# KC-decoder/Multimodal-Brain-Pattern-Identification_XAI

Hardware: AMD Instinct MI355X
Metric: samples/sec train (multimodal SpectrogramCNN+EEGNet fusion, B=64/GPU, 4x128x256 spectro + 10000x19 EEG) (higher is better)
Workload: dtype bf16

## Files before the change

multimodal-brain-pattern-identification_xai_amd/csrc/conv3x3_mfma.hip:

```cpp
#include <stdlib.h>
#include "bx_common.h"
#include <string.h>

typedef __attribute__((ext_vector_type(8))) short bf16x8;
typedef __attribute__((ext_vector_type(4))) float f32x4;
typedef unsigned int u32x4 __attribute__((ext_vector_type(4)));
typedef unsigned int u32x2 __attribute__((ext_vector_type(2)));

static inline int mfma_ck(int Ci) { return Ci < 64 ? Ci : 64; }
static inline int mfma_ks(int ck) { return (9 * ck + 31) / 32; }

int bx_conv3x3_mfma_supported(int Ci, int Co, int dtype) {
  if (dtype != BX_BF16) return 0;
  if (!(Ci == 8 || Ci == 16 || Ci == 32 || (Ci >= 64 && Ci % 64 == 0))) return 0;
  return (Co >= 16 && Co % 16 == 0) || (Co == 8 && (Ci == 16 || Ci == 32));
}
static inline int mfma_ow(int O_p) { return O_p < 16 ? 16 : O_p; }
extern "C" size_t bx_conv3x3_packed_mfma_bytes(int I_p, int O_p) {
  if (!bx_conv3x3_mfma_supported(I_p, O_p, BX_BF16)) return 0;
  const int ck = mfma_ck(I_p);
  return (size_t)(I_p / ck) * mfma_ks(ck) * mfma_ow(O_p) * 32 * sizeof(bf16_t);
}

__global__ void k_pack_mfma(const float* __restrict__ w, bf16_t* __restrict__ wp, int Cout, int Cin, int I_p, int O_p, int tf,
// ... 173 lines not shown

__device__ __forceinline__ unsigned char relu_bits(u32x2 v) {
  const uint32_t h[4] = {v.x & 0xffffu, v.x >> 16, v.y & 0xffffu, v.y >> 16};
  unsigned b = 0;
#pragma unroll
  for (int r = 0; r < 4; ++r) b |= (h[r] != 0u && h[r] < 0x8000u) ? (1u << r) : 0u;
  return (unsigned char)b;
}
template <int CTRL> __device__ __forceinline__ float dpp16(float v) {
  return __int_as_float(__builtin_amdgcn_update_dpp(0, __float_as_int(v), CTRL, 0xf, 0xf, false));
}
__device__ __forceinline__ float row16_sum(float v) {
  v += dpp16<0xB1>(v); v += dpp16<0x4E>(v); v += dpp16<0x124>(v); v += dpp16<0x128>(v);
  return v;
}
template <int MP, int NC, int TPR, typename PixFn>
__device__ __forceinline__ void conv_pool_tiles(const f32x4 (&q)[MP][NC], const BxConvPoolEpi& pe, const __amdgpu_buffer_rsrc_t& pres, int Co,
                                                int co_base, PixFn pix, float (&st)[2][NC][4]) {
  const int lane = threadIdx.x & 63, g = lane >> 4, li = lane & 15;
  const __amdgpu_buffer_rsrc_t rres = __builtin_amdgcn_make_buffer_rsrc(pe.route, 0, pe.route ? pe.route_bytes : 0u, 0x00020000);
#pragma unroll
  for (int i = 0; i < MP; ++i) {
    if ((i / TPR) % 2) continue;
    int bimg, oy, ox;
    pix(i, bimg, oy, ox);
    const bool own = !(li & 1) && (oy >> 1) < pe.Ho && (ox >> 1) < pe.Wo;
    const uint32_t po = own ? (uint32_t)(((((bimg * pe.Ho + (oy >> 1)) * pe.Wo + (ox >> 1)) * Co) + co_base + 4 * g) * 2) : 0x80000000u;
#pragma unroll
    for (int n = 0; n < NC; ++n) {
      float v[4];
      uint32_t code = 0;
#pragma unroll
      for (int r = 0; r < 4; ++r) {
        const float t0 = q[i][n][r], b0 = q[i + TPR][n][r];
        const float t1 = dpp16<0xB1>(t0), b1 = dpp16<0xB1>(b0);
        v[r] = pe.pool == BX_POOL_MAX ? fmaxf(fmaxf(t0, t1), fmaxf(b0, b1)) : 0.25f * (t0 + t1 + b0 + b1);
        if (pe.route) {
          uint32_t nib;
          if (pe.pool == BX_POOL_MAX) {
            nib = t0 == v[r] ? 1u : t1 == v[r] ? 2u : b0 == v[r] ? 4u : 8u;
            nib = v[r] > 0.f ? nib : 0u;
          } else {
            nib = (t0 > 0.f ? 1u : 0u) | (t1 > 0.f ? 2u : 0u) | (b0 > 0.f ? 4u : 0u) | (b1 > 0.f ? 8u : 0u);
          }
          code |= nib << (4 * r);
        }
      }
      const uint32_t lo = pack2bf(v[0], v[1]), hi = pack2bf(v[2], v[3]);
      __builtin_amdgcn_raw_buffer_store_b64((u32x2){lo, hi}, pres, po + (uint32_t)(n * 32), 0, 0);
      __builtin_amdgcn_raw_buffer_store_b16((short)code, rres, own ? (po >> 2) + (uint32_t)(n * 8) : 0x80000000u, 0, 0);
      if (own) {
        const float w[4] = {__uint_as_float(lo << 16), __uint_as_float(lo & 0xffff0000u), __uint_as_float(hi << 16), __uint_as_float(hi & 0xffff0000u)};
#pragma unroll
        for (int r = 0; r < 4; ++r) { st[0][n][r] += w[r]; st[1][n][r] += w[r] * w[r]; }
      }
    }
  }
}
template <int NC>
__device__ __forceinline__ void conv_pool_finish(float (&st)[2][NC][4], const BxConvPoolEpi& pe, int co_base, char* lds) {
  if (!pe.want_stats) return;
  const int wave = threadIdx.x >> 6, lane = threadIdx.x & 63, g = lane >> 4, li = lane & 15;
  constexpr int CW = NC * 16;
#pragma unroll
  for (int k = 0; k < 2; ++k)
// ... 169 lines not shown
      for (int n = 0; n < NC; ++n) {
        const float v[4] = {fmaxf(acc[i][n][0] + bz[n].x, 0.f), fmaxf(acc[i][n][1] + bz[n].y, 0.f), fmaxf(acc[i][n][2] + bz[n].z, 0.f),
                            fmaxf(acc[i][n][3] + bz[n].w, 0.f)};
        const u32x2 out = {pack2bf(v[0], v[1]), pack2bf(v[2], v[3])};
        if (pe.store_y) __builtin_amdgcn_raw_buffer_store_b64(out, yres, offs[i][n], 0, 0);
        acc[i][n] = (f32x4){__uint_as_float(out.x << 16), __uint_as_float(out.x & 0xffff0000u), __uint_as_float(out.y << 16),
                            __uint_as_float(out.y & 0xffff0000u)};
      }
    const uint32_t p_bytes = (uint32_t)((size_t)gx / (tiles_x * tiles_y) * IMGS * pe.Ho * pe.Wo * Co * 2);
    const __amdgpu_buffer_rsrc_t pres = __builtin_amdgcn_make_buffer_rsrc(pe.pooled, 0, p_bytes, 0x00020000);
    float st[2][NC][4];
#pragma unroll
    for (int n = 0; n < NC; ++n)
#pragma unroll
      for (int r = 0; r < 4; ++r) st[0][n][r] = st[1][n][r] = 0.f;
    conv_pool_tiles<MP, NC, TPR>(acc, pe, pres, Co, co_base, [&](int i, int& bimg, int& oy, int& ox) {
      const int t = wave * MP + i, img = t / TPI, tl = t % TPI;
      bimg = b + img; oy = y0 + tl / TPR; ox = x0 + (tl % TPR) * 16 + li;
    }, st);
    conv_pool_finish<NC>(st, pe, co_base, lds);
    return;
  }
  if (mask_src) {
    if (mbits) {
#pragma unroll
      for (int i = 0; i < MP; ++i)
#pragma unroll
        for (int n = 0; n < NCW; ++n) mk[i][n].x = __builtin_amdgcn_raw_buffer_load_b8(mres, offs[i][n] >> 3, 0, 0);
    } else {
#pragma unroll
      for (int i = 0; i < MP; ++i)
#pragma unroll
        for (int n = 0; n < NCW; ++n) mk[i][n] = __builtin_amdgcn_raw_buffer_load_b64(mres, offs[i][n], 0, 0);
// ... 169 lines not shown
      for (int n = 0; n < NCW; ++n) {
        const float v[4] = {fmaxf(acc[i][n][0] + bz[n].x, 0.f), fmaxf(acc[i][n][1] + bz[n].y, 0.f), fmaxf(acc[i][n][2] + bz[n].z, 0.f),
                            fmaxf(acc[i][n][3] + bz[n].w, 0.f)};
        const u32x2 out = {pack2bf(v[0], v[1]), pack2bf(v[2], v[3])};
        if (pe.store_y) __builtin_amdgcn_raw_buffer_store_b64(out, yres, offs[i] + (uint32_t)(n * 32), 0, 0);
        acc[i][n] = (f32x4){__uint_as_float(out.x << 16), __uint_as_float(out.x & 0xffff0000u), __uint_as_float(out.y << 16),
                            __uint_as_float(out.y & 0xffff0000u)};
      }
    const uint32_t p_bytes = (uint32_t)((size_t)gridDim.x / (tiles_x * tiles_y) * IMGS * pe.Ho * pe.Wo * Co * 2);
    const __amdgpu_buffer_rsrc_t pres = __builtin_amdgcn_make_buffer_rsrc(pe.pooled, 0, p_bytes, 0x00020000);
    float st[2][NCW][4];
#pragma unroll
    for (int n = 0; n < NCW; ++n)
#pragma unroll
      for (int r = 0; r < 4; ++r) st[0][n][r] = st[1][n][r] = 0.f;
    conv_pool_tiles<MPT, NCW, TPR>(acc, pe, pres, Co, co_base, [&](int i, int& bimg, int& oy, int& ox) {
      const int img = i / TPI, tl = i % TPI;
      bimg = b + img; oy = y0 + tl / TPR; ox = x0 + (tl % TPR) * 16 + li;
    }, st);
    if (pe.want_stats) {
#pragma unroll
      for (int k = 0; k < 2; ++k)
#pragma unroll
        for (int n = 0; n < NCW; ++n)
#pragma unroll
          for (int r = 0; r < 4; ++r) st[k][n][r] = row16_sum(st[k][n][r]);
      if (li == 0) {
#pragma unroll
        for (int k = 0; k < 2; ++k)
#pragma unroll
          for (int n = 0; n < NCW; ++n)
            *reinterpret_cast<float4*>(pe.tree.rows + ((size_t)blockIdx.x * 2 + k) * pe.tree.ld + co_base + n * 16 + 4 * g) =
                make_float4(st[k][n][0], st[k][n][1], st[k][n][2], st[k][n][3]);
// ... 30 lines not shown
        for (int r = 0; r < 4; ++r) v[r] = (mm[r] != 0u && mm[r] < 0x8000u) ? v[r] : 0.f;
      }
      if (addend) {
        const u32x2 a2 = ad[i][n];
        v[0] += __uint_as_float(a2.x << 16); v[1] += __uint_as_float(a2.x & 0xffff0000u);
        v[2] += __uint_as_float(a2.y << 16); v[3] += __uint_as_float(a2.y & 0xffff0000u);
      }
      const u32x2 out = {pack2bf(v[0], v[1]), pack2bf(v[2], v[3])};
      __builtin_amdgcn_raw_buffer_store_b64(out, yres, offs[i] + (uint32_t)(n * 32), 0, 0);
    }
  }
  BX_CSTAMP(6);
}

template <int CK, int NC, int TW, bool POOL = false, bool C8 = false>
__global__ __launch_bounds__(256, (CK == 16 && NC == 1 && TW == 32 && !POOL) ? 4 : 1) void k_conv_mfma_p(const bf16_t* __restrict__ x, const bf16_t* __restrict__ wp, const float* __restrict__ bias,
    const bf16_t* __restrict__ mask_src, const bf16_t* __restrict__ addend, bf16_t* __restrict__ y,
    int H, int W, int Co, int relu, int tiles_x, int tiles_y, int ntiles, uint32_t x_bytes, BxConvPoolEpi pe, WgradRedList red, int nred) {
  constexpr int TH = 8, HWID = TW + 2, HH = TH + 2, CKB = CK * 2, NCH = CK / 8, KS = (9 * CK + 31) / 32;
  constexpr int MP = TH * TW / 64, TPR = TW / 16;
  constexpr int NU = HH * HWID * NCH, NR = (NU + 255) / 256;
  extern __shared__ __attribute__((aligned(16))) char lds[];
  if ((int)blockIdx.x < nred) {
    if (blockIdx.y == 0) wgrad_reduce_list(red, (int)blockIdx.x, reinterpret_cast<float4*>(lds));
    return;
  }
  const int first_tile = (int)blockIdx.x - nred, tile_stride = (int)gridDim.x - nred;
  const int co_base = blockIdx.y * (NC * 16);
  const int wave = threadIdx.x >> 6, lane = threadIdx.x & 63, g = lane >> 4, li = lane & 15;
  uint4 rv[NR];
  const __amdgpu_buffer_rsrc_t xres = __builtin_amdgcn_make_buffer_rsrc((void*)x, 0, x_bytes, 0x00020000);
// ... 22 lines not shown
  const uint32_t y_bytes = (uint32_t)((size_t)(ntiles / (tiles_x * tiles_y)) * H * W * Co * 2);
  const __amdgpu_buffer_rsrc_t yres = __builtin_amdgcn_make_buffer_rsrc((void*)y, 0, y_bytes, 0x00020000);
  const bool mbits = (relu & 2) != 0;
  const __amdgpu_buffer_rsrc_t mres = __builtin_amdgcn_make_buffer_rsrc((void*)(mask_src ? mask_src : y), 0, mbits ? y_bytes / 8 : y_bytes, 0x00020000);
  const __amdgpu_buffer_rsrc_t ares = __builtin_amdgcn_make_buffer_rsrc((void*)(addend ? addend : y), 0, y_bytes, 0x00020000);
  const uint32_t lane_rel = (uint32_t)((li * Co + co_base + 4 * g) * 2);
  const int Cw = C8 ? 16 : Co;
  const bool ch_ok = C8 ? g < 2 : true;
  float4 bz[NC];
#pragma unroll
  for (int n = 0; n < NC; ++n)
    bz[n] = bias && ch_ok ? *reinterpret_cast<const float4*>(bias + co_base + n * 16 + 4 * g) : make_float4(0.f, 0.f, 0.f, 0.f);
  if (first_tile < ntiles) fetch(first_tile);
  float st[2][NC][4];
  __amdgpu_buffer_rsrc_t pres = yres;
  if constexpr (POOL) {
    conv_pool_transpose_w1x1(pe, Co);
    pres = __builtin_amdgcn_make_buffer_rsrc(pe.pooled, 0, (uint32_t)((size_t)(ntiles / (tiles_x * tiles_y)) * pe.Ho * pe.Wo * Co * 2), 0x00020000);
#pragma unroll
    for (int n = 0; n < NC; ++n)
#pragma unroll
      for (int r = 0; r < 4; ++r) st[0][n][r] = st[1][n][r] = 0.f;
  }
  for (int tile = first_tile; tile < ntiles; tile += tile_stride) {
    const int tx = tile % tiles_x, ty = (tile / tiles_x) % tiles_y, b = tile / (tiles_x * tiles_y);
    const int y0 = ty * TH, x0 = tx * TW;
    __syncthreads();
#pragma unroll
    for (int k = 0; k < NR; ++k) {
      const int u = threadIdx.x + k * 256;
      if (u < NU) {
// ... 25 lines not shown
      const int c = (q0 % CK) / 8;
      const bool valid = tap < 9;
      if (!valid) tap = 0;
      const int dy = tap / 3, dx = tap - 3 * dy;
#pragma unroll
      for (int i = 0; i < MP; ++i) {
        const int t = wave * MP + i;
        const int p = (t / TPR + dy) * HWID + (t % TPR) * 16 + li + dx;
        bf16x8 bv = *reinterpret_cast<const bf16x8*>(lds + p * CKB + 16 * lds_chunk<CK>(c, p));
        if (!valid) bv = (bf16x8){0, 0, 0, 0, 0, 0, 0, 0};
#pragma unroll
        for (int n = 0; n < NC; ++n) acc[i][n] = __builtin_amdgcn_mfma_f32_16x16x32_bf16(a[s % 3][n], bv, acc[i][n], 0, 0, 0);
      }
    }
    const uint32_t tile_o = (uint32_t)((((b * H + y0) * W + x0) * Co) * 2) + lane_rel;
    uint32_t offs[MP][NC];
    u32x2 mk[MP][NC], ad[MP][NC];
#pragma unroll
    for (int i = 0; i < MP; ++i) {
      const int t = wave * MP + i;
      const int oy = y0 + t / TPR, ox = x0 + (t % TPR) * 16 + li;
      const bool inb = oy < H && ox < W && ch_ok;
      const uint32_t orow = tile_o + (uint32_t)((((t / TPR) * W + (t % TPR) * 16) * Co) * 2);
#pragma unroll
      for (int n = 0; n < NC; ++n) offs[i][n] = inb ? orow + (uint32_t)(n * 32) : 0x80000000u;
    }
    if constexpr (POOL) {
#pragma unroll
      for (int i = 0; i < MP; ++i)
#pragma unroll
        for (int n = 0; n < NC; ++n) {
          const float v[4] = {fmaxf(acc[i][n][0] + bz[n].x, 0.f), fmaxf(acc[i][n][1] + bz[n].y, 0.f), fmaxf(acc[i][n][2] + bz[n].z, 0.f),
                              fmaxf(acc[i][n][3] + bz[n].w, 0.f)};
          const u32x2 out = {pack2bf(v[0], v[1]), pack2bf(v[2], v[3])};
          if (pe.store_y) __builtin_amdgcn_raw_buffer_store_b64(out, yres, offs[i][n], 0, 0);
          acc[i][n] = (f32x4){__uint_as_float(out.x << 16), __uint_as_float(out.x & 0xffff0000u), __uint_as_float(out.y << 16),
                              __uint_as_float(out.y & 0xffff0000u)};
        }
      conv_pool_tiles<MP, NC, TPR>(acc, pe, pres, Co, co_base, [&](int i, int& bimg, int& oy, int& ox) {
        const int t = wave * MP + i;
        bimg = b; oy = y0 + t / TPR; ox = x0 + (t % TPR) * 16 + li;
      }, st);
      continue;
    }
    if (mask_src) {
      if (mbits) {
#pragma unroll
        for (int i = 0; i < MP; ++i)
#pragma unroll
          for (int n = 0; n < NC; ++n) mk[i][n].x = __builtin_amdgcn_raw_buffer_load_b8(mres, offs[i][n] >> 3, 0, 0);
      } else {
#pragma unroll
        for (int i = 0; i < MP; ++i)
#pragma unroll
          for (int n = 0; n < NC; ++n) mk[i][n] = __builtin_amdgcn_raw_buffer_load_b64(mres, offs[i][n], 0, 0);
      }
    }
    if (addend) {
// ... 22 lines not shown
          for (int r = 0; r < 4; ++r) v[r] = (mm[r] != 0u && mm[r] < 0x8000u) ? v[r] : 0.f;
        }
        if (addend) {
          const u32x2 a2 = ad[i][n];
          v[0] += __uint_as_float(a2.x << 16); v[1] += __uint_as_float(a2.x & 0xffff0000u);
          v[2] += __uint_as_float(a2.y << 16); v[3] += __uint_as_float(a2.y & 0xffff0000u);
        }
        const u32x2 out = {pack2bf(v[0], v[1]), pack2bf(v[2], v[3])};
        __builtin_amdgcn_raw_buffer_store_b64(out, yres, offs[i][n], 0, 0);
      }
    }
  }
  if constexpr (POOL) conv_pool_finish<NC>(st, pe, co_base, lds);
}

template <bool STORE1>
__global__ __launch_bounds__(256, 4) void k_conv12_mfma(const bf16_t* __restrict__ x, const bf16_t* __restrict__ wp1, const float* __restrict__ bias1,
    const bf16_t* __restrict__ wp2, const float* __restrict__ bias2, bf16_t* __restrict__ y1, bf16_t* __restrict__ y2,
    unsigned char* __restrict__ m1, unsigned char* __restrict__ m2, int H, int W, int tiles_x, int tiles_y, int ntiles, uint32_t x_bytes) {
  constexpr int TH = 8, TW = 32, XW = TW + 4, XH = TH + 4, YW = TW + 2, YH = TH + 2, NX = XH * XW, NY = YH * YW;
  constexpr int NR = (NX + 255) / 256, NT1 = (NY + 15) / 16, MP = TH * TW / 64, TPR = TW / 16, KS1 = 3, KS2 = 5;
  extern __shared__ __attribute__((aligned(16))) char lds[];
  char* xs = lds;
  char* y1s = lds + NX * 16;
  const int wave = threadIdx.x >> 6, lane = threadIdx.x & 63, g = lane >> 4, li = lane & 15;
  const __amdgpu_buffer_rsrc_t xres = __builtin_amdgcn_make_buffer_rsrc((void*)x, 0, x_bytes, 0x00020000);
  int hpy[NR], hpx[NR];
  uint32_t hrel[NR];
#pragma unroll
  for (int k = 0; k < NR; ++k) {
    const int u = threadIdx.x + k * 256;
    hpy[k] = u < NX ? u / XW - 2 : -100000;
    hpx[k] = u % XW - 2;
    hrel[k] = (uint32_t)(((u / XW - 2) * W + (u % XW - 2)) * 8) * 2u;
  }
  uint4 rv[NR];
  auto fetch = [&](int tile) {
    const int tx = tile % tiles_x, ty = (tile / tiles_x) % tiles_y, b = tile / (tiles_x * tiles_y);
    const int y0 = ty * TH, x0 = tx * TW;
    const uint32_t tbase = (uint32_t)(((b * H + y0) * W + x0) * 8) * 2u;
#pragma unroll
    for (int k = 0; k < NR; ++k) {
      const bool ok = (unsigned)(y0 + hpy[k]) < (unsigned)H && (unsigned)(x0 + hpx[k]) < (unsigned)W;
      const u32x4 v = __builtin_amdgcn_raw_buffer_load_b128(xres, ok ? tbase + hrel[k] : 0x80000000u, 0, 0);
      rv[k] = make_uint4(v.x, v.y, v.z, v.w);
    }
  };
  const uint32_t y_bytes = (uint32_t)((size_t)(ntiles / (tiles_x * tiles_y)) * H * W * 16 * 2);
  const __amdgpu_buffer_rsrc_t y1res = __builtin_amdgcn_make_buffer_rsrc((void*)(STORE1 ? y1 : y2), 0, y_bytes, 0x00020000);
  const __amdgpu_buffer_rsrc_t y2res = __builtin_amdgcn_make_buffer_rsrc((void*)y2, 0, y_bytes, 0x00020000);
  const __amdgpu_buffer_rsrc_t m1res = __builtin_amdgcn_make_buffer_rsrc((void*)(STORE1 && m1 ? (void*)m1 : (void*)y2), 0, STORE1 && m1 ? y_bytes / 8 : 0u, 0x00020000);
  const __amdgpu_buffer_rsrc_t m2res = __builtin_amdgcn_make_buffer_rsrc((void*)(STORE1 && m2 ? (void*)m2 : (void*)y2), 0, STORE1 && m2 ? y_bytes / 8 : 0u, 0x00020000);
  bf16x8 a1[KS1], a2[KS2];
#pragma unroll
  for (int s = 0; s < KS1; ++s) a1[s] = *reinterpret_cast<const bf16x8*>(wp1 + ((size_t)s * 16 + li) * 32 + 8 * g);
#pragma unroll
  for (int s = 0; s < KS2; ++s) a2[s] = *reinterpret_cast<const bf16x8*>(wp2 + ((size_t)s * 16 + li) * 32 + 8 * g);
  const float4 b1z = *reinterpret_cast<const float4*>(bias1 + 4 * g), b2z = *reinterpret_cast<const float4*>(bias2 + 4 * g);
  const int first_tile = (int)blockIdx.x, tile_stride = (int)gridDim.x;
  if (first_tile < ntiles) fetch(first_tile);
  for (int tile = first_tile; tile < ntiles; tile += tile_stride) {
    const int tx = tile % tiles_x, ty = (tile / tiles_x) % tiles_y, b = tile / (tiles_x * tiles_y);
    const int y0 = ty * TH, x0 = tx * TW;
    __syncthreads();
#pragma unroll
    for (int k = 0; k < NR; ++k) {
      const int u = threadIdx.x + k * 256;
      if (u < NX) *reinterpret_cast<uint4*>(xs + u * 16) = rv[k];
    }
    __syncthreads();
    if (tile + tile_stride < ntiles) fetch(tile + tile_stride);
#pragma unroll 2
    for (int it = 0; it < (NT1 + 3) / 4; ++it) {
      const int t = wave + 4 * it;
      if (t >= NT1) break;
      const int p = 16 * t + li, pc = p < NY ? p : NY - 1;
      const int r = pc / YW, c = pc - r * YW;
      f32x4 acc = {0.f, 0.f, 0.f, 0.f};
#pragma unroll
      for (int s = 0; s < KS1; ++s) {
        int tap = 4 * s + g;
        const bool valid = tap < 9;
        if (!valid) tap = 0;
        const int dy = tap / 3, dx = tap - 3 * dy;
        bf16x8 bv = *reinterpret_cast<const bf16x8*>(xs + ((r + dy) * XW + c + dx) * 16);
        if (!valid) bv = (bf16x8){0, 0, 0, 0, 0, 0, 0, 0};
        acc = __builtin_amdgcn_mfma_f32_16x16x32_bf16(a1[s], bv, acc, 0, 0, 0);
      }
      const int iy = y0 - 1 + r, ix = x0 - 1 + c;
      const bool inside = p < NY && (unsigned)iy < (unsigned)H && (unsigned)ix < (unsigned)W;
      const float v0 = inside ? fmaxf(acc[0] + b1z.x, 0.f) : 0.f, v1 = inside ? fmaxf(acc[1] + b1z.y, 0.f) : 0.f;
      const float v2 = inside ? fmaxf(acc[2] + b1z.z, 0.f) : 0.f, v3 = inside ? fmaxf(acc[3] + b1z.w, 0.f) : 0.f;
      const u32x2 out = {pack2bf(v0, v1), pack2bf(v2, v3)};
      if (p < NY) *reinterpret_cast<u32x2*>(y1s + p * 32 + 8 * g) = out;
      if constexpr (STORE1) {
        const bool own = inside && r >= 1 && r <= TH && c >= 1 && c <= TW;
        const uint32_t off = own ? (uint32_t)((((b * H + iy) * W + ix) * 16 + 4 * g) * 2) : 0x80000000u;
        __builtin_amdgcn_raw_buffer_store_b64(out, y1res, off, 0, 0);
        __builtin_amdgcn_raw_buffer_store_b8(relu_bits(out), m1res, off >> 3, 0, 0);
      }
    }
    __syncthreads();
    f32x4 acc2[MP];
#pragma unroll
    for (int i = 0; i < MP; ++i) acc2[i] = (f32x4){0.f, 0.f, 0.f, 0.f};
#pragma unroll
    for (int s = 0; s < KS2; ++s) {
      const int q0 = s * 32 + 8 * g;
      int tap = q0 / 16;
      const int c8 = (q0 % 16) / 8;
      const bool valid = tap < 9;
      if (!valid) tap = 0;
      const int dy = tap / 3, dx = tap - 3 * dy;
#pragma unroll
      for (int i = 0; i < MP; ++i) {
        const int t = wave * MP + i;
        const int p = (t / TPR + dy) * YW + (t % TPR) * 16 + li + dx;
        bf16x8 bv = *reinterpret_cast<const bf16x8*>(y1s + p * 32 + 16 * c8);
        if (!valid) bv = (bf16x8){0, 0, 0, 0, 0, 0, 0, 0};
        acc2[i] = __builtin_amdgcn_mfma_f32_16x16x32_bf16(a2[s], bv, acc2[i], 0, 0, 0);
      }
    }
#pragma unroll
    for (int i = 0; i < MP; ++i) {
      const int t = wave * MP + i;
      const int oy = y0 + t / TPR, ox = x0 + (t % TPR) * 16 + li;
      const bool inb = oy < H && ox < W;
      const uint32_t off = inb ? (uint32_t)((((b * H + oy) * W + ox) * 16 + 4 * g) * 2) : 0x80000000u;
      const u32x2 out = {pack2bf(fmaxf(acc2[i][0] + b2z.x, 0.f), fmaxf(acc2[i][1] + b2z.y, 0.f)),
                         pack2bf(fmaxf(acc2[i][2] + b2z.z, 0.f), fmaxf(acc2[i][3] + b2z.w, 0.f))};
      __builtin_amdgcn_raw_buffer_store_b64(out, y2res, off, 0, 0);
      if constexpr (STORE1) __builtin_amdgcn_raw_buffer_store_b8(relu_bits(out), m2res, off >> 3, 0, 0);
    }
  }
}
template <int C0, int C1, bool STORE1>
__global__ __launch_bounds__(256, C1 <= 32 ? 4 : 2) void k_conv12b_mfma(const bf16_t* __restrict__ x, const bf16_t* __restrict__ wp1, const float* __restrict__ bias1,
    const bf16_t* __restrict__ wp2, const float* __restrict__ bias2, bf16_t* __restrict__ y1, bf16_t* __restrict__ y2,
    unsigned char* __restrict__ m1, unsigned char* __restrict__ m2, int H, int W, int tiles_x, int tiles_y, int ntiles, uint32_t x_bytes) {
  constexpr int TH = 8, TW = 32, XW = TW + 4, XH = TH + 4, YW = TW + 2, YH = TH + 2, NX = XH * XW, NY = YH * YW;
  constexpr int NCH0 = C0 / 8, XB = C0 * 2, YB = C1 * 2, NU = NX * NCH0, NR = (NU + 255) / 256, NT1 = (NY + 15) / 16, MP = TH * TW / 64, TPR = TW / 16;
  constexpr int KS1 = (9 * C0 + 31) / 32, KS2 = (9 * C1 + 31) / 32, NC = C1 / 16;
  extern __shared__ __attribute__((aligned(16))) char lds[];
  char* xs = lds;
  char* y1s = lds + NX * XB;
  const int wave = threadIdx.x >> 6, lane = threadIdx.x & 63, g = lane >> 4, li = lane & 15;
  const __amdgpu_buffer_rsrc_t xres = __builtin_amdgcn_make_buffer_rsrc((void*)x, 0, x_bytes, 0x00020000);
  const uint32_t y_bytes = (uint32_t)((size_t)(ntiles / (tiles_x * tiles_y)) * H * W * C1 * 2);
  const __amdgpu_buffer_rsrc_t y1res = __builtin_amdgcn_make_buffer_rsrc((void*)(STORE1 ? y1 : y2), 0, y_bytes, 0x00020000);
  const __amdgpu_buffer_rsrc_t y2res = __builtin_amdgcn_make_buffer_rsrc((void*)y2, 0, y_bytes, 0x00020000);
  const __amdgpu_buffer_rsrc_t m1res = __builtin_amdgcn_make_buffer_rsrc((void*)(STORE1 && m1 ? (void*)m1 : (void*)y2), 0, STORE1 && m1 ? y_bytes / 8 : 0u, 0x00020000);
  const __amdgpu_buffer_rsrc_t m2res = __builtin_amdgcn_make_buffer_rsrc((void*)(STORE1 && m2 ? (void*)m2 : (void*)y2), 0, STORE1 && m2 ? y_bytes / 8 : 0u, 0x00020000);
  const int tile = (int)blockIdx.x;
  const int tx = tile % tiles_x, ty = (tile / tiles_x) % tiles_y, b = tile / (tiles_x * tiles_y);
  const int y0 = ty * TH, x0 = tx * TW;
  {
    const uint32_t tbase = (uint32_t)(((b * H + y0) * W + x0) * C0) * 2u;
// ... 47 lines not shown
#pragma unroll
      for (int n = 0; n < NC; ++n) acc[n] = __builtin_amdgcn_mfma_f32_16x16x32_bf16(a1[s % 3][n], bv, acc[n], 0, 0, 0);
    }
    const int iy = y0 - 1 + r, ix = x0 - 1 + c;
    const bool inside = p < NY && (unsigned)iy < (unsigned)H && (unsigned)ix < (unsigned)W;
    const bool own = inside && r >= 1 && r <= TH && c >= 1 && c <= TW;
    const uint32_t goff = own ? (uint32_t)((((b * H + iy) * W + ix) * C1 + 4 * g) * 2) : 0x80000000u;
#pragma unroll
    for (int n = 0; n < NC; ++n) {
      const float v0 = inside ? fmaxf(acc[n][0] + b1z[n].x, 0.f) : 0.f, v1 = inside ? fmaxf(acc[n][1] + b1z[n].y, 0.f) : 0.f;
      const float v2 = inside ? fmaxf(acc[n][2] + b1z[n].z, 0.f) : 0.f, v3 = inside ? fmaxf(acc[n][3] + b1z[n].w, 0.f) : 0.f;
      const u32x2 out = {pack2bf(v0, v1), pack2bf(v2, v3)};
      if (p < NY) *reinterpret_cast<u32x2*>(y1s + p * YB + 16 * lds_chunk<C1>(2 * n + (g >> 1), p) + 8 * (g & 1)) = out;
      if constexpr (STORE1) {
        __builtin_amdgcn_raw_buffer_store_b64(out, y1res, own ? goff + (uint32_t)(n * 32) : 0x80000000u, 0, 0);
        __builtin_amdgcn_raw_buffer_store_b8(relu_bits(out), m1res, own ? (goff + (uint32_t)(n * 32)) >> 3 : 0x80000000u, 0, 0);
      }
    }
  }
  __syncthreads();
  f32x4 acc2[MP][NC];
#pragma unroll
  for (int i = 0; i < MP; ++i)
#pragma unroll
    for (int n = 0; n < NC; ++n) acc2[i][n] = (f32x4){0.f, 0.f, 0.f, 0.f};
  bf16x8 a2[3][NC];
  auto load_a2 = [&](int s_, bf16x8 (&dst)[NC]) {
#pragma unroll
    for (int n = 0; n < NC; ++n) dst[n] = *reinterpret_cast<const bf16x8*>(wp2 + ((size_t)s_ * C1 + n * 16 + li) * 32 + 8 * g);
  };
  load_a2(0, a2[0]);
// ... 17 lines not shown
#pragma unroll
      for (int n = 0; n < NC; ++n) acc2[i][n] = __builtin_amdgcn_mfma_f32_16x16x32_bf16(a2[s % 3][n], bv, acc2[i][n], 0, 0, 0);
    }
  }
#pragma unroll
  for (int i = 0; i < MP; ++i) {
    const int t = wave * MP + i;
    const int oy = y0 + t / TPR, ox = x0 + (t % TPR) * 16 + li;
    const bool inb = oy < H && ox < W;
    const uint32_t off = inb ? (uint32_t)((((b * H + oy) * W + ox) * C1 + 4 * g) * 2) : 0x80000000u;
#pragma unroll
    for (int n = 0; n < NC; ++n) {
      const u32x2 out = {pack2bf(fmaxf(acc2[i][n][0] + b2z[n].x, 0.f), fmaxf(acc2[i][n][1] + b2z[n].y, 0.f)),
                         pack2bf(fmaxf(acc2[i][n][2] + b2z[n].z, 0.f), fmaxf(acc2[i][n][3] + b2z[n].w, 0.f))};
      __builtin_amdgcn_raw_buffer_store_b64(out, y2res, inb ? off + (uint32_t)(n * 32) : 0x80000000u, 0, 0);
      if constexpr (STORE1) __builtin_amdgcn_raw_buffer_store_b8(relu_bits(out), m2res, inb ? (off + (uint32_t)(n * 32)) >> 3 : 0x80000000u, 0, 0);
    }
  }
}
extern "C" int bx_conv3x3_pair_supported(int C0_p, int C1, int C2, int dtype) {
  return dtype == BX_BF16 && ((C0_p == 8 && C1 == 16 && C2 == 16) || (C0_p == 16 && C1 == 32 && C2 == 32) ||
                              (C0_p == 32 && C1 == 64 && C2 == 64));
}
extern "C" int bx_conv3x3_pair(const void* x, const void* packed1_mfma, const float* bias1, const void* packed2_mfma, const float* bias2,
                               void* y1, void* y2, unsigned char* mask1, unsigned char* mask2, int B, int H, int W, int C0_p, int C1, int C2,
                               int dtype, bxStream stream) {
  BX_REQUIRE(y1 || (!mask1 && !mask2), "bx_conv3x3_pair: the ReLU bit masks are written together with y1 (training passes)");
  BX_REQUIRE(x && packed1_mfma && bias1 && packed2_mfma && bias2 && y2 && B > 0 && H > 0 && W > 0, "bx_conv3x3_pair: bad arguments");
  BX_REQUIRE(bx_conv3x3_pair_supported(C0_p, C1, C2, dtype), "bx_conv3x3_pair: built for bf16 storage, 8 (padded) -> 16 -> 16, 16 -> 32 -> 32 or 32 -> 64 -> 64 channels (got %d -> %d -> %d)",
             C0_p, C1, C2);
  BX_REQUIRE((size_t)B * H * W * C1 * 2 < ((size_t)1 << 31), "bx_conv3x3_pair: an activation tensor of 2 GiB or more is not supported");
  const int tiles_x = (W + 31) / 32, tiles_y = (H + 7) / 8;
  const long long ntiles = (long long)tiles_x * tiles_y * B;
  BX_REQUIRE(ntiles < (1ll << 31), "bx_conv3x3_pair: too many tiles");
  constexpr int gx_cap = 2048;
  const int gx = ntiles < gx_cap ? (int)ntiles : gx_cap;
  if (C1 >= 32) {
    const size_t lds2 = (size_t)12 * 36 * C0_p * 2 + (size_t)10 * 34 * C1 * 2;
    const uint32_t xb2 = (uint32_t)((size_t)B * H * W * C0_p * 2);
    auto go = [&](auto kern) -> int {
      static bool attr_done = false;
      if (lds2 > 64 * 1024 && !attr_done) {
        if (hipFuncSetAttribute((const void*)kern, hipFuncAttributeMaxDynamicSharedMemorySize, (int)lds2) != hipSuccess)
          BX_FAIL(BX_EHIP, "bx_conv3x3_pair: cannot reserve %zu bytes of LDS", lds2);
        attr_done = true;
      }
      hipLaunchKernelGGL(kern, dim3((unsigned)ntiles), dim3(256), lds2, (hipStream_t)stream, (const bf16_t*)x, (const bf16_t*)packed1_mfma, bias1,
                         (const bf16_t*)packed2_mfma, bias2, (bf16_t*)y1, (bf16_t*)y2, y1 ? mask1 : (unsigned char*)nullptr,
                         y1 ? mask2 : (unsigned char*)nullptr, H, W, tiles_x, tiles_y, (int)ntiles, xb2);
      BX_CHECK_LAUNCH("bx_conv3x3_pair (stages 2-3)");
      return BX_OK;
    };
    if (C1 == 32) return y1 ? go(k_conv12b_mfma<16, 32, true>) : go(k_conv12b_mfma<16, 32, false>);
    return y1 ? go(k_conv12b_mfma<32, 64, true>) : go(k_conv12b_mfma<32, 64, false>);
  }
  const size_t lds = (size_t)12 * 36 * 16 + (size_t)10 * 34 * 32;
  const uint32_t xb = (uint32_t)((size_t)B * H * W * 8 * 2);
  if (y1)
    hipLaunchKernelGGL((k_conv12_mfma<true>), dim3((unsigned)gx), dim3(256), lds, (hipStream_t)stream, (const bf16_t*)x, (const bf16_t*)packed1_mfma, bias1,
                       (const bf16_t*)packed2_mfma, bias2, (bf16_t*)y1, (bf16_t*)y2, mask1, mask2, H, W, tiles_x, tiles_y, (int)ntiles, xb);
  else
    hipLaunchKernelGGL((k_conv12_mfma<false>), dim3((unsigned)gx), dim3(256), lds, (hipStream_t)stream, (const bf16_t*)x, (const bf16_t*)packed1_mfma, bias1,
                       (const bf16_t*)packed2_mfma, bias2, (bf16_t*)nullptr, (bf16_t*)y2, (unsigned char*)nullptr, (unsigned char*)nullptr, H, W, tiles_x, tiles_y, (int)ntiles, xb);
  BX_CHECK_LAUNCH("bx_conv3x3_pair");
  return BX_OK;
}

template <int NC>
static int pool_tree_shape(BxConvPoolEpi* pe, int grid_x, int ygroups, int Co) {
  pe->tree.nrows = grid_x; pe->tree.Cw = NC * 16; pe->tree.ld = Co;
  bx_stat_tree_shape(grid_x, &pe->tree.G, &pe->tree.ngroups);
  if (!pe->want_stats) return BX_OK;
  if (grid_x > pe->tree_max_rows) pe->tree.cnt = nullptr;
  BX_REQUIRE((size_t)grid_x * 2 * Co <= pe->rows_cap_floats, "bx_conv3x3(pooled): %d partial rows exceed the workspace", grid_x);
  BX_REQUIRE(!pe->tree.cnt || ygroups * (pe->tree.ngroups + 1) <= pe->cnt_cap_words, "bx_conv3x3(pooled): %d x %d reduction groups exceed the sync words",
             ygroups, pe->tree.ngroups);
  return BX_OK;
// ... 1080 lines not shown
```

Before: 49620.

## Specialise pooled conv epilogue and streamline fused conv pair addressing

Splits the pooled-conv epilogue into template variants for pool type and routing, so the common small-channel case drops runtime branches and the unused route stores. That variant also gets 4-wave launch bounds to allow more blocks per CU. Pooled output offsets are precomputed per lane, and output offsets are now computed at each store instead of being held in a live array. The fused conv1-conv2 kernel hoists tap offsets, steps row/column and global offsets incrementally, and moves the tile base into the buffer-store scalar offset. A new MASKS template flag skips ReLU bitmask stores when no masks are requested; the trade-off is more kernel instantiations and register pressure that could cause spills under the tighter launch bound.

```diff
diff --git a/multimodal-brain-pattern-identification_xai_amd/csrc/conv3x3_mfma.hip b/multimodal-brain-pattern-identification_xai_amd/csrc/conv3x3_mfma.hip
--- a/multimodal-brain-pattern-identification_xai_amd/csrc/conv3x3_mfma.hip
+++ b/multimodal-brain-pattern-identification_xai_amd/csrc/conv3x3_mfma.hip
@@ -211,18 +211,22 @@
   v += dpp16<0xB1>(v); v += dpp16<0x4E>(v); v += dpp16<0x124>(v); v += dpp16<0x128>(v);
   return v;
 }
-template <int MP, int NC, int TPR, typename PixFn>
-__device__ __forceinline__ void conv_pool_tiles(const f32x4 (&q)[MP][NC], const BxConvPoolEpi& pe, const __amdgpu_buffer_rsrc_t& pres, int Co,
-                                                int co_base, PixFn pix, float (&st)[2][NC][4]) {
+__device__ __forceinline__ void conv_pool_po(const BxConvPoolEpi& pe, int Co, int co_base, int bimg, int oy, int ox, bool& own, uint32_t& po) {
   const int lane = threadIdx.x & 63, g = lane >> 4, li = lane & 15;
+  own = !(li & 1) && (oy >> 1) < pe.Ho && (ox >> 1) < pe.Wo;
+  po = own ? (uint32_t)(((((bimg * pe.Ho + (oy >> 1)) * pe.Wo + (ox >> 1)) * Co) + co_base + 4 * g) * 2) : 0x80000000u;
+}
+template <int MP, int NC, int TPR, int PM = -1, int RT = -1, typename PoFn>
+__device__ __forceinline__ void conv_pool_tiles(const f32x4 (&q)[MP][NC], const BxConvPoolEpi& pe, const __amdgpu_buffer_rsrc_t& pres,
+                                                PoFn pofn, float (&st)[2][NC][4]) {
+  const bool pmax = PM < 0 ? pe.pool == BX_POOL_MAX : PM == 1, nibbles = RT < 0 ? pe.route != nullptr : RT == 1;
   const __amdgpu_buffer_rsrc_t rres = __builtin_amdgcn_make_buffer_rsrc(pe.route, 0, pe.route ? pe.route_bytes : 0u, 0x00020000);
 #pragma unroll
   for (int i = 0; i < MP; ++i) {
     if ((i / TPR) % 2) continue;
-    int bimg, oy, ox;
-    pix(i, bimg, oy, ox);
-    const bool own = !(li & 1) && (oy >> 1) < pe.Ho && (ox >> 1) < pe.Wo;
-    const uint32_t po = own ? (uint32_t)(((((bimg * pe.Ho + (oy >> 1)) * pe.Wo + (ox >> 1)) * Co) + co_base + 4 * g) * 2) : 0x80000000u;
+    bool own;
+    uint32_t po;
+    pofn(i, own, po);
 #pragma unroll
     for (int n = 0; n < NC; ++n) {
       float v[4];
@@ -231,11 +235,13 @@
       for (int r = 0; r < 4; ++r) {
         const float t0 = q[i][n][r], b0 = q[i + TPR][n][r];
         const float t1 = dpp16<0xB1>(t0), b1 = dpp16<0xB1>(b0);
-        v[r] = pe.pool == BX_POOL_MAX ? fmaxf(fmaxf(t0, t1), fmaxf(b0, b1)) : 0.25f * (t0 + t1 + b0 + b1);
-        if (pe.route) {
+        v[r] = pmax ? fmaxf(fmaxf(t0, t1), fmaxf(b0, b1)) : 0.25f * (t0 + t1 + b0 + b1);
+        if (nibbles) {
           uint32_t nib;
-          if (pe.pool == BX_POOL_MAX) {
-            nib = t0 == v[r] ? 1u : t1 == v[r] ? 2u : b0 == v[r] ? 4u : 8u;
+          if (pmax) {
+            nib = b0 == v[r] ? 4u : 8u;
+            nib = t1 == v[r] ? 2u : nib;
+            nib = t0 == v[r] ? 1u : nib;
             nib = v[r] > 0.f ? nib : 0u;
           } else {
             nib = (t0 > 0.f ? 1u : 0u) | (t1 > 0.f ? 2u : 0u) | (b0 > 0.f ? 4u : 0u) | (b1 > 0.f ? 8u : 0u);
@@ -245,7 +251,7 @@
       }
       const uint32_t lo = pack2bf(v[0], v[1]), hi = pack2bf(v[2], v[3]);
       __builtin_amdgcn_raw_buffer_store_b64((u32x2){lo, hi}, pres, po + (uint32_t)(n * 32), 0, 0);
-      __builtin_amdgcn_raw_buffer_store_b16((short)code, rres, own ? (po >> 2) + (uint32_t)(n * 8) : 0x80000000u, 0, 0);
+      if (RT != 0) __builtin_amdgcn_raw_buffer_store_b16((short)code, rres, own ? (po >> 2) + (uint32_t)(n * 8) : 0x80000000u, 0, 0);
       if (own) {
         const float w[4] = {__uint_as_float(lo << 16), __uint_as_float(lo & 0xffff0000u), __uint_as_float(hi << 16), __uint_as_float(hi & 0xffff0000u)};
 #pragma unroll
@@ -445,9 +451,9 @@
     for (int n = 0; n < NC; ++n)
 #pragma unroll
       for (int r = 0; r < 4; ++r) st[0][n][r] = st[1][n][r] = 0.f;
-    conv_pool_tiles<MP, NC, TPR>(acc, pe, pres, Co, co_base, [&](int i, int& bimg, int& oy, int& ox) {
+    conv_pool_tiles<MP, NC, TPR>(acc, pe, pres, [&](int i, bool& own, uint32_t& po) {
       const int t = wave * MP + i, img = t / TPI, tl = t % TPI;
-      bimg = b + img; oy = y0 + tl / TPR; ox = x0 + (tl % TPR) * 16 + li;
+      conv_pool_po(pe, Co, co_base, b + img, y0 + tl / TPR, x0 + (tl % TPR) * 16 + li, own, po);
     }, st);
     conv_pool_finish<NC>(st, pe, co_base, lds);
     return;
@@ -647,9 +653,9 @@
     for (int n = 0; n < NCW; ++n)
 #pragma unroll
       for (int r = 0; r < 4; ++r) st[0][n][r] = st[1][n][r] = 0.f;
-    conv_pool_tiles<MPT, NCW, TPR>(acc, pe, pres, Co, co_base, [&](int i, int& bimg, int& oy, int& ox) {
+    conv_pool_tiles<MPT, NCW, TPR>(acc, pe, pres, [&](int i, bool& own, uint32_t& po) {
       const int img = i / TPI, tl = i % TPI;
-      bimg = b + img; oy = y0 + tl / TPR; ox = x0 + (tl % TPR) * 16 + li;
+      conv_pool_po(pe, Co, co_base, b + img, y0 + tl / TPR, x0 + (tl % TPR) * 16 + li, own, po);
     }, st);
     if (pe.want_stats) {
 #pragma unroll
@@ -710,7 +716,7 @@
 }
 
 template <int CK, int NC, int TW, bool POOL = false, bool C8 = false>
-__global__ __launch_bounds__(256, (CK == 16 && NC == 1 && TW == 32 && !POOL) ? 4 : 1) void k_conv_mfma_p(const bf16_t* __restrict__ x, const bf16_t* __restrict__ wp, const float* __restrict__ bias,
+__global__ __launch_bounds__(256, (CK == 16 && NC == 1 && TW == 32) ? 4 : 1) void k_conv_mfma_p(const bf16_t* __restrict__ x, const bf16_t* __restrict__ wp, const float* __restrict__ bias,
     const bf16_t* __restrict__ mask_src, const bf16_t* __restrict__ addend, bf16_t* __restrict__ y,
     int H, int W, int Co, int relu, int tiles_x, int tiles_y, int ntiles, uint32_t x_bytes, BxConvPoolEpi pe, WgradRedList red, int nred) {
   constexpr int TH = 8, HWID = TW + 2, HH = TH + 2, CKB = CK * 2, NCH = CK / 8, KS = (9 * CK + 31) / 32;
@@ -763,7 +769,16 @@
   if (first_tile < ntiles) fetch(first_tile);
   float st[2][NC][4];
   __amdgpu_buffer_rsrc_t pres = yres;
+  constexpr bool POOL_SPEC = POOL && CK == 16 && NC == 1 && TW == 32;
+  const int prow = (wave * MP) / TPR / 2;
+  int pcol[TPR];
+  uint32_t prel[TPR];
   if constexpr (POOL) {
+#pragma unroll
+    for (int j = 0; j < TPR; ++j) {
+      pcol[j] = (j * 16 + li) >> 1;
+      prel[j] = (uint32_t)((((prow * pe.Wo + pcol[j]) * Co) + co_base + 4 * g) * 2);
+    }
     conv_pool_transpose_w1x1(pe, Co);
     pres = __builtin_amdgcn_make_buffer_rsrc(pe.pooled, 0, (uint32_t)((size_t)(ntiles / (tiles_x * tiles_y)) * pe.Ho * pe.Wo * Co * 2), 0x00020000);
 #pragma unroll
@@ -819,17 +834,12 @@
       }
     }
     const uint32_t tile_o = (uint32_t)((((b * H + y0) * W + x0) * Co) * 2) + lane_rel;
-    uint32_t offs[MP][NC];
-    u32x2 mk[MP][NC], ad[MP][NC];
-#pragma unroll
-    for (int i = 0; i < MP; ++i) {
+    auto y_off = [&](int i, bool& inb) -> uint32_t {
       const int t = wave * MP + i;
       const int oy = y0 + t / TPR, ox = x0 + (t % TPR) * 16 + li;
-      const bool inb = oy < H && ox < W && ch_ok;
-      const uint32_t orow = tile_o + (uint32_t)((((t / TPR) * W + (t % TPR) * 16) * Co) * 2);
-#pragma unroll
-      for (int n = 0; n < NC; ++n) offs[i][n] = inb ? orow + (uint32_t)(n * 32) : 0x80000000u;
-    }
+      inb = oy < H && ox < W && ch_ok;
+      return tile_o + (uint32_t)((((t / TPR) * W + (t % TPR) * 16) * Co) * 2);
+    };
     if constexpr (POOL) {
 #pragma unroll
       for (int i = 0; i < MP; ++i)
@@ -838,15 +848,41 @@
           const float v[4] = {fmaxf(acc[i][n][0] + bz[n].x, 0.f), fmaxf(acc[i][n][1] + bz[n].y, 0.f), fmaxf(acc[i][n][2] + bz[n].z, 0.f),
                               fmaxf(acc[i][n][3] + bz[n].w, 0.f)};
           const u32x2 out = {pack2bf(v[0], v[1]), pack2bf(v[2], v[3])};
-          if (pe.store_y) __builtin_amdgcn_raw_buffer_store_b64(out, yres, offs[i][n], 0, 0);
+          if (pe.store_y) {
+            bool inb;
+            const uint32_t orow = y_off(i, inb);
+            __builtin_amdgcn_raw_buffer_store_b64(out, yres, inb ? orow + (uint32_t)(n * 32) : 0x80000000u, 0, 0);
+          }
           acc[i][n] = (f32x4){__uint_as_float(out.x << 16), __uint_as_float(out.x & 0xffff0000u), __uint_as_float(out.y << 16),
                               __uint_as_float(out.y & 0xffff0000u)};
         }
-      conv_pool_tiles<MP, NC, TPR>(acc, pe, pres, Co, co_base, [&](int i, int& bimg, int& oy, int& ox) {
-        const int t = wave * MP + i;
-        bimg = b; oy = y0 + t / TPR; ox = x0 + (t % TPR) * 16 + li;
-      }, st);
+      const uint32_t pbase = (uint32_t)(((((b * pe.Ho + (y0 >> 1)) * pe.Wo + (x0 >> 1)) * Co)) * 2);
+      const int hleft = pe.Ho - (y0 >> 1), wleft = pe.Wo - (x0 >> 1);
+      auto pofn = [&](int i, bool& own, uint32_t& po) {
+        own = !(li & 1) && prow < hleft && pcol[i % TPR] < wleft;
+        po = own ? pbase + prel[i % TPR] : 0x80000000u;
+      };
+      if constexpr (POOL_SPEC) {
+        if (pe.pool == BX_POOL_MAX) {
+          if (pe.route) conv_pool_tiles<MP, NC, TPR, 1, 1>(acc, pe, pres, pofn, st);
+          else conv_pool_tiles<MP, NC, TPR, 1, 0>(acc, pe, pres, pofn, st);
+        } else {
+          if (pe.route) conv_pool_tiles<MP, NC, TPR, 0, 1>(acc, pe, pres, pofn, st);
+          else conv_pool_tiles<MP, NC, TPR, 0, 0>(acc, pe, pres, pofn, st);
+        }
+      } else {
+        conv_pool_tiles<MP, NC, TPR>(acc, pe, pres, pofn, st);
+      }
       continue;
+    }
+    uint32_t offs[MP][NC];
+    u32x2 mk[MP][NC], ad[MP][NC];
+#pragma unroll
+    for (int i = 0; i < MP; ++i) {
+      bool inb;
+      const uint32_t orow = y_off(i, inb);
+#pragma unroll
+      for (int n = 0; n < NC; ++n) offs[i][n] = inb ? orow + (uint32_t)(n * 32) : 0x80000000u;
     }
     if (mask_src) {
       if (mbits) {
@@ -899,16 +935,18 @@
   if constexpr (POOL) conv_pool_finish<NC>(st, pe, co_base, lds);
 }
 
-template <bool STORE1>
+template <bool STORE1, bool MASKS>
 __global__ __launch_bounds__(256, 4) void k_conv12_mfma(const bf16_t* __restrict__ x, const bf16_t* __restrict__ wp1, const float* __restrict__ bias1,
     const bf16_t* __restrict__ wp2, const float* __restrict__ bias2, bf16_t* __restrict__ y1, bf16_t* __restrict__ y2,
     unsigned char* __restrict__ m1, unsigned char* __restrict__ m2, int H, int W, int tiles_x, int tiles_y, int ntiles, uint32_t x_bytes) {
   constexpr int TH = 8, TW = 32, XW = TW + 4, XH = TH + 4, YW = TW + 2, YH = TH + 2, NX = XH * XW, NY = YH * YW;
   constexpr int NR = (NX + 255) / 256, NT1 = (NY + 15) / 16, MP = TH * TW / 64, TPR = TW / 16, KS1 = 3, KS2 = 5;
+  static_assert(STORE1 || !MASKS, "the ReLU bit masks are written together with y1");
   extern __shared__ __attribute__((aligned(16))) char lds[];
   char* xs = lds;
   char* y1s = lds + NX * 16;
-  const int wave = threadIdx.x >> 6, lane = threadIdx.x & 63, g = lane >> 4, li = lane & 15;
+  const int wave = __builtin_amdgcn_readfirstlane((int)(threadIdx.x >> 6));
+  const int lane = threadIdx.x & 63, g = lane >> 4, li = lane & 15;
   const __amdgpu_buffer_rsrc_t xres = __builtin_amdgcn_make_buffer_rsrc((void*)x, 0, x_bytes, 0x00020000);
   int hpy[NR], hpx[NR];
   uint32_t hrel[NR];
@@ -936,6 +974,19 @@
   const __amdgpu_buffer_rsrc_t y2res = __builtin_amdgcn_make_buffer_rsrc((void*)y2, 0, y_bytes, 0x00020000);
   const __amdgpu_buffer_rsrc_t m1res = __builtin_amdgcn_make_buffer_rsrc((void*)(STORE1 && m1 ? (void*)m1 : (void*)y2), 0, STORE1 && m1 ? y_bytes / 8 : 0u, 0x00020000);
   const __amdgpu_buffer_rsrc_t m2res = __builtin_amdgcn_make_buffer_rsrc((void*)(STORE1 && m2 ? (void*)m2 : (void*)y2), 0, STORE1 && m2 ? y_bytes / 8 : 0u, 0x00020000);
+  const int ph0 = 16 * wave + li, hr0 = ph0 / YW, hc0 = ph0 - hr0 * YW;
+  uint32_t tapo[KS1];
+#pragma unroll
+  for (int s = 0; s < KS1; ++s) {
+    const int tap = 4 * s + g < 9 ? 4 * s + g : 0, dy = tap / 3, dx = tap - 3 * dy;
+    tapo[s] = (uint32_t)((dy * XW + dx) * 16);
+  }
+  const uint32_t y1w0 = (uint32_t)(ph0 * 32 + 8 * g);
+  const uint32_t rel1_0 = (uint32_t)((((hr0 - 1) * W + hc0 - 1) * 16 + 4 * g) * 2);
+  const uint32_t rel1s = (uint32_t)((W + 30) * 32), rel1w = (uint32_t)((2 * W + 30 - YW) * 32);
+  uint32_t rel2[MP];
+#pragma unroll
+  for (int i = 0; i < MP; ++i) rel2[i] = (uint32_t)((((wave * MP + i) / TPR * W + (i % TPR) * 16 + li) * 16 + 4 * g) * 2);
   bf16x8 a1[KS1], a2[KS2];
 #pragma unroll
   for (int s = 0; s < KS1; ++s) a1[s] = *reinterpret_cast<const bf16x8*>(wp1 + ((size_t)s * 16 + li) * 32 + 8 * g);
@@ -955,36 +1006,44 @@
     }
     __syncthreads();
     if (tile + tile_stride < ntiles) fetch(tile + tile_stride);
-#pragma unroll 2
-    for (int it = 0; it < (NT1 + 3) / 4; ++it) {
-      const int t = wave + 4 * it;
-      if (t >= NT1) break;
-      const int p = 16 * t + li, pc = p < NY ? p : NY - 1;
-      const int r = pc / YW, c = pc - r * YW;
+    const uint32_t tile_o = (uint32_t)((((b * H + y0) * W + x0) * 16) * 2);
+    int r = hr0, c = hc0;
+    uint32_t rel = rel1_0;
+    static_assert(NT1 == 22, "rounds 0..4 are whole tiles of every wave; round 5 is tile 20 or the ragged tile 21 (waves 0 and 1)");
+    auto round = [&](int it, auto ragged) {
+      const bool live = decltype(ragged)::value ? r < YH : true;
+      const uint32_t xp = live ? __umul24((unsigned)r, (unsigned)XW) + (unsigned)c : 0u;
       f32x4 acc = {0.f, 0.f, 0.f, 0.f};
 #pragma unroll
       for (int s = 0; s < KS1; ++s) {
-        int tap = 4 * s + g;
-        const bool valid = tap < 9;
-        if (!valid) tap = 0;
-        const int dy = tap / 3, dx = tap - 3 * dy;
-        bf16x8 bv = *reinterpret_cast<const bf16x8*>(xs + ((r + dy) * XW + c + dx) * 16);
+        const bool valid = 4 * s + g < 9;
+        bf16x8 bv = *reinterpret_cast<const bf16x8*>(xs + ((xp << 4) + tapo[s]));
         if (!valid) bv = (bf16x8){0, 0, 0, 0, 0, 0, 0, 0};
         acc = __builtin_amdgcn_mfma_f32_16x16x32_bf16(a1[s], bv, acc, 0, 0, 0);
       }
       const int iy = y0 - 1 + r, ix = x0 - 1 + c;
-      const bool inside = p < NY && (unsigned)iy < (unsigned)H && (unsigned)ix < (unsigned)W;
+      const bool inside = live && (unsigned)iy < (unsigned)H && (unsigned)ix < (unsigned)W;
       const float v0 = inside ? fmaxf(acc[0] + b1z.x, 0.f) : 0.f, v1 = inside ? fmaxf(acc[1] + b1z.y, 0.f) : 0.f;
       const float v2 = inside ? fmaxf(acc[2] + b1z.z, 0.f) : 0.f, v3 = inside ? fmaxf(acc[3] + b1z.w, 0.f) : 0.f;
       const u32x2 out = {pack2bf(v0, v1), pack2bf(v2, v3)};
-      if (p < NY) *reinterpret_cast<u32x2*>(y1s + p * 32 + 8 * g) = out;
+      if (live) *reinterpret_cast<u32x2*>(y1s + y1w0 + it * (64 * 32)) = out;
       if constexpr (STORE1) {
-        const bool own = inside && r >= 1 && r <= TH && c >= 1 && c <= TW;
-        const uint32_t off = own ? (uint32_t)((((b * H + iy) * W + ix) * 16 + 4 * g) * 2) : 0x80000000u;
-        __builtin_amdgcn_raw_buffer_store_b64(out, y1res, off, 0, 0);
-        __builtin_amdgcn_raw_buffer_store_b8(relu_bits(out), m1res, off >> 3, 0, 0);
-      }
-    }
+        const bool own = inside & ((unsigned)(r - 1) < (unsigned)TH) & ((unsigned)(c - 1) < (unsigned)TW);
+        __builtin_amdgcn_raw_buffer_store_b64(out, y1res, own ? rel : 0x80000000u, tile_o, 0);
+        if constexpr (MASKS) __builtin_amdgcn_raw_buffer_store_b8(relu_bits(out), m1res, own ? rel >> 3 : 0x80000000u, tile_o >> 3, 0);
+      }
+      const bool wrap = c >= YW - 30;
+      c += wrap ? 30 - YW : 30;
+      r += wrap ? 2 : 1;
+      if constexpr (STORE1) rel += wrap ? rel1w : rel1s;
+    };
+#pragma unroll 1
+    for (int it = 0; it < 4; it += 2) {
+      round(it, std::false_type{});
+      round(it + 1, std::false_type{});
+    }
+    round(4, std::false_type{});
+    if (wave + 20 < NT1) round(5, std::true_type{});
     __syncthreads();
     f32x4 acc2[MP];
 #pragma unroll
@@ -1011,21 +1070,21 @@
       const int t = wave * MP + i;
       const int oy = y0 + t / TPR, ox = x0 + (t % TPR) * 16 + li;
       const bool inb = oy < H && ox < W;
-      const uint32_t off = inb ? (uint32_t)((((b * H + oy) * W + ox) * 16 + 4 * g) * 2) : 0x80000000u;
       const u32x2 out = {pack2bf(fmaxf(acc2[i][0] + b2z.x, 0.f), fmaxf(acc2[i][1] + b2z.y, 0.f)),
                          pack2bf(fmaxf(acc2[i][2] + b2z.z, 0.f), fmaxf(acc2[i][3] + b2z.w, 0.f))};
-      __builtin_amdgcn_raw_buffer_store_b64(out, y2res, off, 0, 0);
-      if constexpr (STORE1) __builtin_amdgcn_raw_buffer_store_b8(relu_bits(out), m2res, off >> 3, 0, 0);
-    }
-  }
-}
-template <int C0, int C1, bool STORE1>
+      __builtin_amdgcn_raw_buffer_store_b64(out, y2res, inb ? rel2[i] : 0x80000000u, tile_o, 0);
+      if constexpr (MASKS) __builtin_amdgcn_raw_buffer_store_b8(relu_bits(out), m2res, inb ? rel2[i] >> 3 : 0x80000000u, tile_o >> 3, 0);
+    }
+  }
+}
+template <int C0, int C1, bool STORE1, bool MASKS>
 __global__ __launch_bounds__(256, C1 <= 32 ? 4 : 2) void k_conv12b_mfma(const bf16_t* __restrict__ x, const bf16_t* __restrict__ wp1, const float* __restrict__ bias1,
     const bf16_t* __restrict__ wp2, const float* __restrict__ bias2, bf16_t* __restrict__ y1, bf16_t* __restrict__ y2,
     unsigned char* __restrict__ m1, unsigned char* __restrict__ m2, int H, int W, int tiles_x, int tiles_y, int ntiles, uint32_t x_bytes) {
   constexpr int TH = 8, TW = 32, XW = TW + 4, XH = TH + 4, YW = TW + 2, YH = TH + 2, NX = XH * XW, NY = YH * YW;
   constexpr int NCH0 = C0 / 8, XB = C0 * 2, YB = C1 * 2, NU = NX * NCH0, NR = (NU + 255) / 256, NT1 = (NY + 15) / 16, MP = TH * TW / 64, TPR = TW / 16;
   constexpr int KS1 = (9 * C0 + 31) / 32, KS2 = (9 * C1 + 31) / 32, NC = C1 / 16;
+  static_assert(STORE1 || !MASKS, "the ReLU bit masks are written together with y1");
   extern __shared__ __attribute__((aligned(16))) char lds[];
   char* xs = lds;
   char* y1s = lds + NX * XB;
@@ -1103,7 +1162,7 @@
       if (p < NY) *reinterpret_cast<u32x2*>(y1s + p * YB + 16 * lds_chunk<C1>(2 * n + (g >> 1), p) + 8 * (g & 1)) = out;
       if constexpr (STORE1) {
         __builtin_amdgcn_raw_buffer_store_b64(out, y1res, own ? goff + (uint32_t)(n * 32) : 0x80000000u, 0, 0);
-        __builtin_amdgcn_raw_buffer_store_b8(relu_bits(out), m1res, own ? (goff + (uint32_t)(n * 32)) >> 3 : 0x80000000u, 0, 0);
+        if constexpr (MASKS) __builtin_amdgcn_raw_buffer_store_b8(relu_bits(out), m1res, own ? (goff + (uint32_t)(n * 32)) >> 3 : 0x80000000u, 0, 0);
       }
     }
   }
@@ -1151,7 +1210,7 @@
       const u32x2 out = {pack2bf(fmaxf(acc2[i][n][0] + b2z[n].x, 0.f), fmaxf(acc2[i][n][1] + b2z[n].y, 0.f)),
                          pack2bf(fmaxf(acc2[i][n][2] + b2z[n].z, 0.f), fmaxf(acc2[i][n][3] + b2z[n].w, 0.f))};
       __builtin_amdgcn_raw_buffer_store_b64(out, y2res, inb ? off + (uint32_t)(n * 32) : 0x80000000u, 0, 0);
-      if constexpr (STORE1) __builtin_amdgcn_raw_buffer_store_b8(relu_bits(out), m2res, inb ? (off + (uint32_t)(n * 32)) >> 3 : 0x80000000u, 0, 0);
+      if constexpr (MASKS) __builtin_amdgcn_raw_buffer_store_b8(relu_bits(out), m2res, inb ? (off + (uint32_t)(n * 32)) >> 3 : 0x80000000u, 0, 0);
     }
   }
 }
@@ -1172,6 +1231,7 @@
   BX_REQUIRE(ntiles < (1ll << 31), "bx_conv3x3_pair: too many tiles");
   constexpr int gx_cap = 2048;
   const int gx = ntiles < gx_cap ? (int)ntiles : gx_cap;
+  const bool masks = mask1 || mask2;
   if (C1 >= 32) {
     const size_t lds2 = (size_t)12 * 36 * C0_p * 2 + (size_t)10 * 34 * C1 * 2;
     const uint32_t xb2 = (uint32_t)((size_t)B * H * W * C0_p * 2);
@@ -1188,16 +1248,19 @@
       BX_CHECK_LAUNCH("bx_conv3x3_pair (stages 2-3)");
       return BX_OK;
     };
-    if (C1 == 32) return y1 ? go(k_conv12b_mfma<16, 32, true>) : go(k_conv12b_mfma<16, 32, false>);
-    return y1 ? go(k_conv12b_mfma<32, 64, true>) : go(k_conv12b_mfma<32, 64, false>);
+    if (C1 == 32) return masks ? go(k_conv12b_mfma<16, 32, true, true>) : y1 ? go(k_conv12b_mfma<16, 32, true, false>) : go(k_conv12b_mfma<16, 32, false, false>);
+    return masks ? go(k_conv12b_mfma<32, 64, true, true>) : y1 ? go(k_conv12b_mfma<32, 64, true, false>) : go(k_conv12b_mfma<32, 64, false, false>);
   }
   const size_t lds = (size_t)12 * 36 * 16 + (size_t)10 * 34 * 32;
   const uint32_t xb = (uint32_t)((size_t)B * H * W * 8 * 2);
-  if (y1)
-    hipLaunchKernelGGL((k_conv12_mfma<true>), dim3((unsigned)gx), dim3(256), lds, (hipStream_t)stream, (const bf16_t*)x, (const bf16_t*)packed1_mfma, bias1,
+  if (masks)
+    hipLaunchKernelGGL((k_conv12_mfma<true, true>), dim3((unsigned)gx), dim3(256), lds, (hipStream_t)stream, (const bf16_t*)x, (const bf16_t*)packed1_mfma, bias1,
                        (const bf16_t*)packed2_mfma, bias2, (bf16_t*)y1, (bf16_t*)y2, mask1, mask2, H, W, tiles_x, tiles_y, (int)ntiles, xb);
+  else if (y1)
+    hipLaunchKernelGGL((k_conv12_mfma<true, false>), dim3((unsigned)gx), dim3(256), lds, (hipStream_t)stream, (const bf16_t*)x, (const bf16_t*)packed1_mfma, bias1,
+                       (const bf16_t*)packed2_mfma, bias2, (bf16_t*)y1, (bf16_t*)y2, (unsigned char*)nullptr, (unsigned char*)nullptr, H, W, tiles_x, tiles_y, (int)ntiles, xb);
   else
-    hipLaunchKernelGGL((k_conv12_mfma<false>), dim3((unsigned)gx), dim3(256), lds, (hipStream_t)stream, (const bf16_t*)x, (const bf16_t*)packed1_mfma, bias1,
+    hipLaunchKernelGGL((k_conv12_mfma<false, false>), dim3((unsigned)gx), dim3(256), lds, (hipStream_t)stream, (const bf16_t*)x, (const bf16_t*)packed1_mfma, bias1,
                        (const bf16_t*)packed2_mfma, bias2, (bf16_t*)nullptr, (bf16_t*)y2, (unsigned char*)nullptr, (unsigned char*)nullptr, H, W, tiles_x, tiles_y, (int)ntiles, xb);
   BX_CHECK_LAUNCH("bx_conv3x3_pair");
   return BX_OK;
```

New measurement: 50100 (median of 6 runs). About the same (+1.0%).
